# hzxie/RMNet

Measured on AMD Instinct MI355X. Metric: frames/sec at 480p, 1 object, T=5 memory; memory-read HBM GB/s vs peak, higher is better.
Workload: dtype f32 convs; memory read = fp16 operands (K, V, q, P rounded to 11 bits), fp32 accumulate (RMNET_BANK_F16): the frame loop's default for clips with one object -- on one-object 480x854 clips whose masks HAVE a boundary (tests/live_fixture.py) mask IoU vs the CPU path 0.99993-0.99997 and foreground logi

## Files before the change

include/rmnet_hip.h:

```cpp
#ifndef RMNET_HIP_H_
#define RMNET_HIP_H_

#include <stddef.h>
#include <stdint.h>

#ifdef __cplusplus
extern "C" {
#endif

#define RMNET_ABI_VERSION 6

enum {
  RMNET_OK = 0,
  RMNET_E_INVALID_ARG = -1,
  RMNET_E_WORKSPACE = -2,
  RMNET_E_LAUNCH = -3,
  RMNET_E_UNSUPPORTED = -4
};

int rmnet_abi_version(void);
const char *rmnet_error_string(int code);

size_t rmnet_region_map_workspace_bytes(int B, int K, int H, int W);
int rmnet_region_map_f32(const float *mask, int B, int K, int H, int W, float prob_threshold,
// ... 49 lines not shown
                           void *ev_start, void *ev_mid, void *ev_end);
size_t rmnet_bank_read_workspace_bytes(int no, int h, int w);
size_t rmnet_bank_read_workspace_bytes_for(int no, int h, int w, int T);
int rmnet_bank_read_f32(void *bank, int no, int Tcap, int h, int w, int T,
                        const float *q_key, const float *q_val, const int32_t *qry_rects,
                        float *mem_val, void *workspace, size_t workspace_bytes, void *stream,
                        void *ev_start, void *ev_mid, void *ev_end);

int rmnet_rect_mask_f32(const float *x, int n, int C, int T, int h, int w, const int32_t *rects,
                        float *y, void *stream);

int rmnet_channel_affine_f32(const float *x, const float *scale, const float *shift,
                             const float *res, const float *res_scale, const float *res_shift,
                             int relu, long long N, int C, long long HW, float *out, void *stream);

int rmnet_affine_relu_maxpool_f32(const float *x, const float *scale, const float *shift, long long N,
                                  int C, int H, int W, float *out, void *stream);

int rmnet_upsample2x_add_f32(const float *x, const float *skip, long long N, int C, int h, int w,
                             float *out, void *stream);

int rmnet_channel_affine_nhwc_f32(const float *x, const float *scale, const float *shift, const float *res, const float *res_scale,
                                  const float *res_shift, int relu, long long rows, int C, float *out, void *stream);
int rmnet_upsample2x_add_nhwc_f32(const float *x, const float *skip, long long N, int C, int h, int w, float *out, void *stream);
int rmnet_affine_relu_maxpool_nhwc_f32(const float *x, const float *scale, const float *shift, long long N, int C, int H, int W,
                                       float *out, void *stream);

#define RMNET_CONV_RELU_IN 1
#define RMNET_CONV_RELU_OUT 2
int rmnet_conv3x3_split_f32(const float *x, const void *wpack, const float *w_unscale, const float *bias, const float *res, int flags,
                            int N, int H, int W, int Cin, float *out, int32_t *range_word, void *stream);

int rmnet_conv3x3_split_lds_f32(const float *x, const void *wpack, const float *w_unscale, const float *bias, const float *res,
                                int flags, int N, int H, int W, int Cin, float *out, int32_t *range_word, void *stream);

int rmnet_conv3x3_rows_f32(const float *x, const void *wpack, const float *w_unscale, const float *bias, const float *res, int flags,
                           int N, int H, int W, int Cin, float *out, int32_t *range_word, void *stream);

int rmnet_conv_split_f32(const float *x, const void *wpack, const float *w_unscale, const float *shift, const float *res, int flags,
                         int N, int H, int W, int Cin, int Cout, int ksize, int stride, float *out, float *out2, int out_split,
                         int32_t *range_word, void *stream);

#define RMNET_CONV_X_SPLIT 4
#define RMNET_CONV_OUT_SPLIT 8
int rmnet_conv_split_pre_f32(const void *x, const void *wpack, const float *w_unscale, const float *shift, const float *res, int flags,
                             int N, int H, int W, int Cin, int Cout, int ksize, int stride, void *out, float *out2, int out_split,
                             int32_t *range_word, void *stream);
int rmnet_split_act_f32(const float *x, long long M, int C, int relu, void *out, int32_t *range_word, void *stream);

int rmnet_conv_rows_pre_f32(const void *x, const void *wpack, const float *w_unscale, const float *shift, const float *res, int flags,
                            int N, int H, int W, int Cin, int Cout, int ksize, int stride, void *out, float *out2, int out_split,
                            int32_t *range_word, void *stream);

int rmnet_stem_split_f32(const float *frame, const float *mask, const float *other, const void *wpack, const float *w_unscale,
                         const float *shift, int N, int H, int W, float *out, int32_t *range_word, void *stream);

int rmnet_flow_stem_f32(const float *img0, const float *img1, long long batch_stride0, long long batch_stride1, const void *wpack,
                        const float *w_unscale, const float *bias, int N, int H, int W, int Hpad, int Wpad, int lh, int lw, float *out, int32_t *range_word, void *stream);

int rmnet_pred_head_f32(const float *x, const float *w, const float *bias, int n, int Hq, int Wq, int C, float *out, void *stream);

#define RMNET_FLOW_RELU 1
#define RMNET_FLOW_LEAKY 2
#define RMNET_FLOW_TRANSPOSED 4
int rmnet_flow_conv_f32(const float *x, int x_ld, const void *wpack, const float *w_unscale, const float *shift, int flags, int N, int H,
                        int W, int Cin, int Cout, int ksize, int stride, float *out, int out_ld, int coff, int32_t *range_word,
                        void *stream);

size_t rmnet_flow_head_workspace_bytes(int N, int H, int W, int Cin);
int rmnet_flow_head_f32(const float *x, int x_ld, const float *wpack, const float *bias, int N, int H, int W, int Cin, float *out,
                        void *workspace, size_t workspace_bytes, void *stream);

int rmnet_flow_up_f32(const float *flow, const float *w, int N, int h, int w_, float *out, int out_ld, int coff, void *stream);

int rmnet_soft_aggregate_f32(const float *dec, const int32_t *obj_begin, int B, int K, int Hp, int Wp,
                             int pad_l, int pad_t, int H, int W, float *logit, float *prob,
                             void *stream);

int rmnet_flow_affine_f32(const float *flow, const float *m1, const float *m2, int H, int W,
                          float *out, void *stream);
size_t rmnet_flow_affine_workspace_bytes(int H, int W);
int rmnet_flow_affine_f32_host(const float *flow_host, const float *m1_host, const float *m2_host,
                               int H, int W, float *out_host, void *workspace,
                               size_t workspace_bytes, void *stream);

#ifdef __cplusplus
}
#endif
#endif
```

rmnet_amd/_lib.py:

```python

import ctypes
import os

_HERE = os.path.dirname(os.path.abspath(__file__))
LIB_PATH = os.environ.get('RMNET_HIP_LIB') or os.path.join(_HERE, 'librmnet_hip.so')

c_f32p = ctypes.c_void_p
c_i32p = ctypes.c_void_p

SIGNATURES = {
    'rmnet_abi_version': (ctypes.c_int, []),
    'rmnet_error_string': (ctypes.c_char_p, [ctypes.c_int]),
    'rmnet_region_map_workspace_bytes': (ctypes.c_size_t, [ctypes.c_int] * 4),
    'rmnet_region_map_f32': (ctypes.c_int, [
        c_f32p, ctypes.c_int, ctypes.c_int, ctypes.c_int, ctypes.c_int, ctypes.c_float, ctypes.c_int,
        ctypes.c_int, c_f32p, c_i32p, c_i32p, ctypes.c_int, ctypes.c_int, ctypes.c_int, ctypes.c_int,
        ctypes.c_int, ctypes.c_void_p, ctypes.c_size_t, ctypes.c_void_p]),
    'rmnet_region_map_warped_f32': (ctypes.c_int, [
        c_f32p, c_f32p, ctypes.c_int, ctypes.c_int, ctypes.c_int, ctypes.c_int, ctypes.c_float, ctypes.c_int,
        ctypes.c_int, c_f32p, c_i32p, c_i32p, ctypes.c_int, ctypes.c_int, ctypes.c_int, ctypes.c_int,
        ctypes.c_int, c_f32p, ctypes.c_void_p, ctypes.c_size_t, ctypes.c_void_p]),
    'rmnet_boxes_to_cell_rects_i32': (ctypes.c_int, [
        c_i32p, ctypes.c_int, ctypes.c_int, ctypes.c_int, ctypes.c_int, ctypes.c_int, ctypes.c_int,
        ctypes.c_int, c_i32p, ctypes.c_void_p]),
# ... 15 lines not shown
        ctypes.c_void_p, ctypes.c_int, ctypes.c_int, ctypes.c_int, ctypes.c_int, ctypes.c_int, c_f32p,
        c_f32p, c_i32p, ctypes.c_void_p]),
    'rmnet_bank_append_f32_at': (ctypes.c_int, [
        ctypes.c_void_p, ctypes.c_int, ctypes.c_int, ctypes.c_int, ctypes.c_int, ctypes.c_int, c_i32p, c_f32p,
        c_f32p, c_i32p, ctypes.c_void_p]),
    'rmnet_bank_read_f32_at': (ctypes.c_int, [
        ctypes.c_void_p, ctypes.c_int, ctypes.c_int, ctypes.c_int, ctypes.c_int, ctypes.c_int, c_i32p, ctypes.c_int, c_f32p,
        c_f32p, c_i32p, c_f32p, ctypes.c_void_p, ctypes.c_size_t, ctypes.c_void_p, ctypes.c_void_p,
        ctypes.c_void_p, ctypes.c_void_p]),
    'rmnet_bank_read_workspace_bytes': (ctypes.c_size_t, [ctypes.c_int] * 3),
    'rmnet_bank_read_workspace_bytes_for': (ctypes.c_size_t, [ctypes.c_int] * 4),
    'rmnet_bank_read_f32': (ctypes.c_int, [
        ctypes.c_void_p, ctypes.c_int, ctypes.c_int, ctypes.c_int, ctypes.c_int, ctypes.c_int, c_f32p,
        c_f32p, c_i32p, c_f32p, ctypes.c_void_p, ctypes.c_size_t, ctypes.c_void_p, ctypes.c_void_p,
        ctypes.c_void_p, ctypes.c_void_p]),
    'rmnet_rect_mask_f32': (ctypes.c_int, [
        c_f32p, ctypes.c_int, ctypes.c_int, ctypes.c_int, ctypes.c_int, ctypes.c_int, c_i32p, c_f32p,
        ctypes.c_void_p]),
    'rmnet_channel_affine_f32': (ctypes.c_int, [
        c_f32p, c_f32p, c_f32p, c_f32p, c_f32p, c_f32p, ctypes.c_int, ctypes.c_longlong, ctypes.c_int,
        ctypes.c_longlong, c_f32p, ctypes.c_void_p]),
    'rmnet_upsample2x_add_f32': (ctypes.c_int, [
        c_f32p, c_f32p, ctypes.c_longlong, ctypes.c_int, ctypes.c_int, ctypes.c_int, c_f32p, ctypes.c_void_p]),
    'rmnet_soft_aggregate_f32': (ctypes.c_int, [
        c_f32p, c_i32p, ctypes.c_int, ctypes.c_int, ctypes.c_int, ctypes.c_int, ctypes.c_int, ctypes.c_int,
        ctypes.c_int, ctypes.c_int, c_f32p, c_f32p, ctypes.c_void_p]),
    'rmnet_affine_relu_maxpool_f32': (ctypes.c_int, [
        c_f32p, c_f32p, c_f32p, ctypes.c_longlong, ctypes.c_int, ctypes.c_int, ctypes.c_int, c_f32p,
        ctypes.c_void_p]),
    'rmnet_channel_affine_nhwc_f32': (ctypes.c_int, [
        c_f32p, c_f32p, c_f32p, c_f32p, c_f32p, c_f32p, ctypes.c_int, ctypes.c_longlong, ctypes.c_int, c_f32p, ctypes.c_void_p]),
    'rmnet_upsample2x_add_nhwc_f32': (ctypes.c_int, [
        c_f32p, c_f32p, ctypes.c_longlong, ctypes.c_int, ctypes.c_int, ctypes.c_int, c_f32p, ctypes.c_void_p]),
    'rmnet_affine_relu_maxpool_nhwc_f32': (ctypes.c_int, [
        c_f32p, c_f32p, c_f32p, ctypes.c_longlong, ctypes.c_int, ctypes.c_int, ctypes.c_int, c_f32p, ctypes.c_void_p]),
    'rmnet_conv3x3_split_f32': (ctypes.c_int, [
        c_f32p, ctypes.c_void_p, c_f32p, c_f32p, c_f32p, ctypes.c_int, ctypes.c_int, ctypes.c_int, ctypes.c_int, ctypes.c_int,
        c_f32p, c_i32p, ctypes.c_void_p]),
    'rmnet_conv3x3_split_lds_f32': (ctypes.c_int, [
        c_f32p, ctypes.c_void_p, c_f32p, c_f32p, c_f32p, ctypes.c_int, ctypes.c_int, ctypes.c_int, ctypes.c_int, ctypes.c_int,
        c_f32p, c_i32p, ctypes.c_void_p]),
    'rmnet_conv3x3_rows_f32': (ctypes.c_int, [
        c_f32p, ctypes.c_void_p, c_f32p, c_f32p, c_f32p, ctypes.c_int, ctypes.c_int, ctypes.c_int, ctypes.c_int, ctypes.c_int,
        c_f32p, c_i32p, ctypes.c_void_p]),
    'rmnet_conv_split_f32': (ctypes.c_int, [
        c_f32p, ctypes.c_void_p, c_f32p, c_f32p, c_f32p, ctypes.c_int, ctypes.c_int, ctypes.c_int, ctypes.c_int, ctypes.c_int,
        ctypes.c_int, ctypes.c_int, ctypes.c_int, c_f32p, c_f32p, ctypes.c_int, c_i32p, ctypes.c_void_p]),
    'rmnet_conv_split_pre_f32': (ctypes.c_int, [
        ctypes.c_void_p, ctypes.c_void_p, c_f32p, c_f32p, c_f32p, ctypes.c_int, ctypes.c_int, ctypes.c_int, ctypes.c_int, ctypes.c_int,
        ctypes.c_int, ctypes.c_int, ctypes.c_int, ctypes.c_void_p, c_f32p, ctypes.c_int, c_i32p, ctypes.c_void_p]),
    'rmnet_conv_rows_pre_f32': (ctypes.c_int, [
        ctypes.c_void_p, ctypes.c_void_p, c_f32p, c_f32p, c_f32p, ctypes.c_int, ctypes.c_int, ctypes.c_int, ctypes.c_int, ctypes.c_int,
        ctypes.c_int, ctypes.c_int, ctypes.c_int, ctypes.c_void_p, c_f32p, ctypes.c_int, c_i32p, ctypes.c_void_p]),
    'rmnet_split_act_f32': (ctypes.c_int, [
        c_f32p, ctypes.c_longlong, ctypes.c_int, ctypes.c_int, ctypes.c_void_p, c_i32p, ctypes.c_void_p]),
    'rmnet_stem_split_f32': (ctypes.c_int, [
        c_f32p, c_f32p, c_f32p, ctypes.c_void_p, c_f32p, c_f32p, ctypes.c_int, ctypes.c_int, ctypes.c_int, c_f32p, c_i32p,
        ctypes.c_void_p]),
    'rmnet_flow_stem_f32': (ctypes.c_int, [
        c_f32p, c_f32p, ctypes.c_longlong, ctypes.c_longlong, ctypes.c_void_p, c_f32p, c_f32p, ctypes.c_int, ctypes.c_int, ctypes.c_int,
        ctypes.c_int, ctypes.c_int, ctypes.c_int, ctypes.c_int, c_f32p, c_i32p, ctypes.c_void_p]),
    'rmnet_pred_head_f32': (ctypes.c_int, [
        c_f32p, c_f32p, c_f32p, ctypes.c_int, ctypes.c_int, ctypes.c_int, ctypes.c_int, c_f32p, ctypes.c_void_p]),
    'rmnet_flow_conv_f32': (ctypes.c_int, [
        c_f32p, ctypes.c_int, ctypes.c_void_p, c_f32p, c_f32p, ctypes.c_int, ctypes.c_int, ctypes.c_int, ctypes.c_int, ctypes.c_int,
        ctypes.c_int, ctypes.c_int, ctypes.c_int, c_f32p, ctypes.c_int, ctypes.c_int, c_i32p, ctypes.c_void_p]),
    'rmnet_flow_head_workspace_bytes': (ctypes.c_size_t, [ctypes.c_int] * 4),
    'rmnet_flow_head_f32': (ctypes.c_int, [
        c_f32p, ctypes.c_int, c_f32p, c_f32p, ctypes.c_int, ctypes.c_int, ctypes.c_int, ctypes.c_int, c_f32p, ctypes.c_void_p,
        ctypes.c_size_t, ctypes.c_void_p]),
    'rmnet_flow_up_f32': (ctypes.c_int, [
        c_f32p, c_f32p, ctypes.c_int, ctypes.c_int, ctypes.c_int, c_f32p, ctypes.c_int, ctypes.c_int, ctypes.c_void_p]),
    'rmnet_flow_affine_f32': (ctypes.c_int, [
        c_f32p, c_f32p, c_f32p, ctypes.c_int, ctypes.c_int, c_f32p, ctypes.c_void_p]),
    'rmnet_flow_affine_workspace_bytes': (ctypes.c_size_t, [ctypes.c_int, ctypes.c_int]),
    'rmnet_flow_affine_f32_host': (ctypes.c_int, [
        ctypes.c_void_p, ctypes.c_void_p, ctypes.c_void_p, ctypes.c_int, ctypes.c_int,
        ctypes.c_void_p, ctypes.c_void_p, ctypes.c_size_t, ctypes.c_void_p]),
}

ABI_VERSION = 6
_lib = None


class RMNetHipError(RuntimeError):
    pass


def load():
    global _lib
    if _lib is not None:
        return _lib
    if not os.path.exists(LIB_PATH):
        raise RMNetHipError(
            'librmnet_hip.so is missing (%s). The HIP kernels are the only implementation of this '
            'path; build them with `python -m rmnet_amd.build`.' % LIB_PATH)
    lib = ctypes.CDLL(LIB_PATH)
    for name, (res, args) in SIGNATURES.items():
        fn = getattr(lib, name)
        fn.restype = res
        fn.argtypes = args
    if lib.rmnet_abi_version() != ABI_VERSION:
        raise RMNetHipError('librmnet_hip.so ABI %d != expected %d' % (lib.rmnet_abi_version(), ABI_VERSION))
    _lib = lib
    return lib

# ... 6 lines not shown
```

rmnet_amd/build.py:

```python

import os
import shutil
import subprocess

HERE = os.path.dirname(os.path.abspath(__file__))
CSRC = os.path.join(HERE, 'csrc')
SOURCES = ['capi.hip', 'region_map.hip', 'flow_affine.hip', 'memory_read.hip', 'bank.hip', 'epilogue.hip', 'conv3x3.hip', 'conv3x3_rows.hip', 'conv_split.hip',
           'conv_rows.hip', 'stem.hip', 'pred_head.hip', 'flow_conv.hip', 'flow_head.hip', 'flow_stem.hip']
LIB = os.path.join(HERE, 'librmnet_hip.so')
ARCH = 'gfx950'


def hipcc_path():
    for cand in (shutil.which('hipcc'), '/opt/rocm/bin/hipcc'):
        if cand and os.path.exists(cand):
            return cand
    raise RuntimeError('hipcc not found: librmnet_hip.so cannot be built')


def dependencies():
    headers = sorted(f for f in os.listdir(CSRC) if f.endswith('.h'))
    return [os.path.join(CSRC, f) for f in SOURCES + headers] + [os.path.join(os.path.dirname(HERE), 'include', 'rmnet_hip.h')]


def needs_build():
    if not os.path.exists(LIB):
        return True
    t = os.path.getmtime(LIB)
    return any(os.path.getmtime(d) > t for d in dependencies())


def build_library(force=False, verbose=False):
    if not force and not needs_build():
        return LIB
    cmd = [hipcc_path(), '--offload-arch=' + ARCH, '-O3', '-std=c++17', '-shared', '-fPIC',
           '-o', LIB] + [os.path.join(CSRC, s) for s in SOURCES]
    if verbose:
        print(' '.join(cmd))
    subprocess.check_call(cmd, cwd=CSRC)
    return LIB


if __name__ == '__main__':
    print(build_library(force=True, verbose=True))
```

rmnet_amd/csrc/conv_rows_core.h:

```cpp
#pragma once

#include <mutex>

#include "common.h"

namespace rmnet {
namespace {

typedef _Float16 half8 __attribute__((ext_vector_type(8)));
typedef _Float16 half4 __attribute__((ext_vector_type(4)));
typedef float f32x4 __attribute__((ext_vector_type(4)));
typedef unsigned int u32x4 __attribute__((ext_vector_type(4)));

constexpr int kKT = 32;
constexpr int kThreads = 512;
constexpr float kActScale = 64.0f;
constexpr float kActUnscale = 1.0f / 64.0f;
constexpr float kF16Max = 65504.0f;
constexpr int kZeroRows = 4;
constexpr int kAhead = 1;

constexpr int rows_image_bytes(int C, int MT) { return (MT + 2 + kZeroRows) * C * 4; }

__device__ inline int swzr(int row, int chunk) { return row * kKT + ((chunk ^ ((row >> 1) & 2)) << 3); }

__device__ inline void split4(const f32x4 v, half4& hi, half4& lo, int& bad, int count = 1) {
#pragma unroll
  for (int e = 0; e < 4; ++e) {
    const float y = v[e] * kActScale;
    bad += !(fabsf(y) <= kF16Max) ? count : 0;
    const float c = fminf(fmaxf(y, -kF16Max), kF16Max);
    const _Float16 h = (_Float16)c;
    hi[e] = h;
    lo[e] = (_Float16)(c - (float)h);
  }
}

inline bool overlap(const void* p, long long pn, const void* q, long long qn) {
  const char* a = reinterpret_cast<const char*>(p);
  const char* b = reinterpret_cast<const char*>(q);
  return a < b + qn && b < a + pn;
}

extern __shared__ __attribute__((aligned(16))) _Float16 rows_lds[];

template <int C, int MT>
struct RowsCore {
  static constexpr int kCB = C / kKT;
  static constexpr int kStaged = MT + 2;
  static constexpr int kPlaneHalves = (kStaged + kZeroRows) * kKT;
  static constexpr int kBlockHalves = 2 * kPlaneHalves;
  static constexpr int kWPlane = C * kKT;
  static_assert(C % kKT == 0 && kCB % 2 == 0 && MT % 128 == 0 && (MT / 128) * kCB == 8, "8 waves of 128 pixels x 32 channels");
  static_assert(kStaged % 4 == 2, "the zero row of a masked lane: (kStaged + (row + 2) % 4) % 4 == row % 4");
  static_assert(kCB * kBlockHalves * 2 == rows_image_bytes(C, MT), "the image");

  int fr, fc, pix;
  unsigned inside[3];
  half8 wa[4], wb[4];
  const half8* wsrc;
  const half8* wlast;
  unsigned wl;
  f32x4 acc[8][2], accx[8][2];

  __device__ __forceinline__ void begin(int tid, int wcol, int pix_, int m1, const half8* wp, int M, int H, int W) {
    fr = tid & 15, fc = (tid & 63) >> 4, pix = pix_;
    if (tid < 16 * 2 * kCB) *reinterpret_cast<half8*>(rows_lds + (tid >> 4) * kPlaneHalves + kStaged * kKT + 8 * (tid & 15)) = half8{0, 0, 0, 0, 0, 0, 0, 0};
    const int HW = H * W;
    inside[0] = inside[1] = inside[2] = 0u;
#pragma unroll
    for (int i = 0; i < 8; ++i) {
      const int m = m1 + 16 * i + fr;
      const bool pin = m < M;
      const int r = (pin ? m : 0) % HW;
      const int ph = r / W, pw = r % W;
      unsigned bits = 0;
#pragma unroll
      for (int t = 0; t < 9; ++t) {
        const int h = ph + t / 3 - 1, w = pw + t % 3 - 1;
        bits |= (pin && h >= 0 && h < H && w >= 0 && w < W ? 1u : 0u) << t;
      }
      inside[i / 3] |= bits << (9 * (i % 3));
    }
    wsrc = wp;
    wlast = wp + (9 * kCB - 1) * (2 * kWPlane / 8);
    wl = (wcol * 32 + fr) * 4 + fc;
#pragma unroll
    for (int i = 0; i < 8; ++i)
#pragma unroll
      for (int j = 0; j < 2; ++j) acc[i][j] = accx[i][j] = f32x4{0.f, 0.f, 0.f, 0.f};
    load_w(wa);
  }

  __device__ __forceinline__ void load_w(half8 (&w)[4]) {
// ... 5 lines not shown
  }

  __device__ __forceinline__ void run_tap(int tap) {
    const int dx1 = tap % 3;
    unsigned ao[8];
#pragma unroll
    for (int i = 0; i < 8; ++i) {
      const bool in = (inside[i / 3] >> (9 * (i % 3) + tap)) & 1;
      const int row = pix + 16 * i + fr + dx1;
      const unsigned real = (unsigned)swzr(row, fc);
      ao[i] = in ? real : (unsigned)((kStaged + ((row + 2) & 3)) * kKT) + (real & (kKT - 1));
    }
    half8 bh[kAhead + 1], bl[kAhead + 1];
    auto frag = [&](int n) __attribute__((always_inline)) {
      const _Float16* p = rows_lds + ao[n & 7] + (n >> 3) * kBlockHalves;
      bh[n % (kAhead + 1)] = *reinterpret_cast<const half8*>(p);
      bl[n % (kAhead + 1)] = *reinterpret_cast<const half8*>(p + kPlaneHalves);
    };
    auto mma = [&](int cb, const half8(&w)[4]) __attribute__((always_inline)) {
#pragma unroll
      for (int i = 0; i < 8; ++i) {
        if (8 * cb + i + kAhead < 8 * kCB) frag(8 * cb + i + kAhead);
        const half8 h = bh[(8 * cb + i) % (kAhead + 1)], l = bl[(8 * cb + i) % (kAhead + 1)];
#pragma unroll
        for (int j = 0; j < 2; ++j) acc[i][j] = __builtin_amdgcn_mfma_f32_16x16x32_f16(w[2 * j], h, acc[i][j], 0, 0, 0);
#pragma unroll
        for (int j = 0; j < 2; ++j) accx[i][j] = __builtin_amdgcn_mfma_f32_16x16x32_f16(w[2 * j], l, accx[i][j], 0, 0, 0);
#pragma unroll
        for (int j = 0; j < 2; ++j) accx[i][j] = __builtin_amdgcn_mfma_f32_16x16x32_f16(w[2 * j + 1], h, accx[i][j], 0, 0, 0);
      }
    };
    auto step = [&](int cb, const half8(&wc)[4], half8(&wn)[4]) __attribute__((always_inline)) {
      __builtin_amdgcn_sched_barrier(0);
      load_w(wn);
      __builtin_amdgcn_sched_barrier(0);
      mma(cb, wc);
#pragma unroll
      for (int i = 0; i < 8; ++i) {
        __builtin_amdgcn_sched_group_barrier(0x100, 2, 0);
        __builtin_amdgcn_sched_group_barrier(0x008, 6, 0);
      }
    };
#pragma unroll
    for (int n = 0; n < kAhead; ++n) frag(n);
#pragma unroll
    for (int cb = 0; cb < kCB; cb += 2) {
      step(cb, wa, wb);
      step(cb + 1, wb, wa);
    }
    __builtin_amdgcn_sched_barrier(0);
  }

  __device__ __forceinline__ void unscale_shift(const float* unscale, const float* shift, int wcol) {
#pragma unroll
    for (int j = 0; j < 2; ++j) {
      const int co = wcol * 32 + j * 16 + 4 * fc;
      const f32x4 us = *reinterpret_cast<const f32x4*>(unscale + co) * kActUnscale;
      const f32x4 b = shift ? *reinterpret_cast<const f32x4*>(shift + co) : f32x4{0.f, 0.f, 0.f, 0.f};
#pragma unroll
      for (int i = 0; i < 8; ++i) acc[i][j] = (acc[i][j] + accx[i][j]) * us + b;
    }
#pragma unroll
    for (int j = 0; j < 2; ++j)
#pragma unroll
      for (int i = 0; i < 8; ++i) asm volatile("" : "+v"(acc[i][j]));
  }
};

template <auto Kernel, int kBytes>
int rows_prepare(hipStream_t st) {
  static std::mutex mu;
  static bool done[64] = {};
  int dev = 0;
  if (hipGetDevice(&dev) != hipSuccess || dev < 0 || dev >= 64) return RMNET_E_LAUNCH;
  std::lock_guard<std::mutex> lock(mu);
  if (done[dev]) return RMNET_OK;
  hipStreamCaptureStatus cs = hipStreamCaptureStatusNone;
  if (hipStreamIsCapturing(st, &cs) != hipSuccess) return RMNET_E_LAUNCH;
  if (cs != hipStreamCaptureStatusNone) return RMNET_E_UNSUPPORTED;
  if (hipFuncSetAttribute(reinterpret_cast<const void*>(Kernel), hipFuncAttributeMaxDynamicSharedMemorySize, kBytes) != hipSuccess)
    return RMNET_E_LAUNCH;
  done[dev] = true;
  return RMNET_OK;
}

}
}
```

rmnet_amd/networks.py:

```python

import torch
import torch.nn.functional as F
from torch import nn


class _Bottleneck(nn.Module):

    def __init__(self, c_in, width, stride, project):
        super().__init__()
        c_out = width * 4
        self.conv1 = nn.Conv2d(c_in, width, 1, bias=False)
        self.bn1 = nn.BatchNorm2d(width)
        self.conv2 = nn.Conv2d(width, width, 3, stride=stride, padding=1, bias=False)
        self.bn2 = nn.BatchNorm2d(width)
        self.conv3 = nn.Conv2d(width, c_out, 1, bias=False)
        self.bn3 = nn.BatchNorm2d(c_out)
        self.relu = nn.ReLU(inplace=True)
        self.downsample = None
        if project:
            self.downsample = nn.Sequential(nn.Conv2d(c_in, c_out, 1, stride=stride, bias=False),
                                            nn.BatchNorm2d(c_out))

    def forward(self, x):
        if getattr(self, '_fused', False) and not self.training and x.is_cuda:
            return self._forward_fused(x)
        skip = x if self.downsample is None else self.downsample(x)
        y = self.relu(self.bn1(self.conv1(x)))
        y = self.relu(self.bn2(self.conv2(y)))
        y = self.bn3(self.conv3(y))
        return self.relu(y + skip)

    def _forward_fused(self, x):
        from . import ops
        if _split_path_ok(self, x, self.conv1, ('full', 'split', 'trunk')):
            x = x.contiguous(memory_format=torch.channels_last)
            rw = ops.conv_range_word(x.device)
            pre = conv_presplit()
            t = ops.conv_split(x, self._wp1, self._wu1, self._b1, ksize=1, relu_out=True, range_word=rw, out_presplit=pre)
            t = ops.conv_split(t, self._wp2, self._wu2, self._b2, ksize=3, stride=self.conv2.stride[0], relu_out=True, range_word=rw,
                               out_presplit=pre and self.conv3.in_channels >= PRESPLIT_MIN_CIN_1X1)
            if self.downsample is None:
                return ops.conv_split(t, self._wp3, self._wu3, self._b3, res=x, ksize=1, relu_out=True, range_word=rw)
            d = ops.conv_split(x, self._wpd, self._wud, self._bd, ksize=1, stride=self.downsample[0].stride[0], range_word=rw)
            return ops.conv_split(t, self._wp3, self._wu3, self._b3, res=d, ksize=1, relu_out=True, out=d, range_word=rw)
        t = self.conv1(x)
        ops.channel_affine(t, self._s1, self._b1, relu=True, out=t)
        t = self.conv2(t)
        ops.channel_affine(t, self._s2, self._b2, relu=True, out=t)
        t = self.conv3(t)
        if self.downsample is None:
            return ops.channel_affine(t, self._s3, self._b3, res=x, relu=True, out=t)
        d = self.downsample[0](x)
        return ops.channel_affine(t, self._s3, self._b3, res=d, res_scale=self._sd, res_shift=self._bd,
                                  relu=True, out=t)


def _stage(c_in, width, n_blocks, stride):
    blocks = [_Bottleneck(c_in, width, stride, project=True)]
    blocks += [_Bottleneck(width * 4, width, 1, project=False) for _ in range(n_blocks - 1)]
    return nn.Sequential(*blocks)


class ResNet50Trunk(nn.Module):

    def __init__(self):
        super().__init__()
        self.conv1 = nn.Conv2d(3, 64, 7, stride=2, padding=3, bias=False)
        self.bn1 = nn.BatchNorm2d(64)
        self.relu = nn.ReLU(inplace=True)
        self.maxpool = nn.MaxPool2d(3, stride=2, padding=1)
        self.layer1 = _stage(64, 64, 3, 1)
        self.layer2 = _stage(256, 128, 4, 2)
        self.layer3 = _stage(512, 256, 6, 2)


def resnet50(pretrained=False):
    return ResNet50Trunk()


class ResBlock(nn.Module):

    def __init__(self, indim, outdim=None, stride=1):
        super().__init__()
        outdim = indim if outdim is None else outdim
        self.downsample = None
        if not (indim == outdim and stride == 1):
            self.downsample = nn.Conv2d(indim, outdim, 3, padding=1, stride=stride)
        self.conv1 = nn.Conv2d(indim, outdim, 3, padding=1, stride=stride)
        self.conv2 = nn.Conv2d(outdim, outdim, 3, padding=1)

    def forward(self, x):
        if getattr(self, '_fused', False) and not self.training and x.is_cuda:
            return self._forward_fused(x)
        r = self.conv2(F.relu(self.conv1(F.relu(x))))
        return (x if self.downsample is None else self.downsample(x)) + r

    def _forward_fused(self, x):
        from . import ops
        c1, c2 = self.conv1, self.conv2
        if self.downsample is None and _split_conv_ok(self, x, c1) and _split_conv_ok(self, x, c2):
            x = x.contiguous(memory_format=torch.channels_last)
            rw = ops.conv_range_word(x.device)
            t = ops.conv3x3_split(x, self._wp1, self._wu1, c1.bias, relu_in=True, relu_out=True, range_word=rw)
            return ops.conv3x3_split(t, self._wp2, self._wu2, c2.bias, res=x, range_word=rw)
        t = F.conv2d(F.relu(x), c1.weight, None, c1.stride, c1.padding)
        ops.channel_affine(t, None, c1.bias, relu=True, out=t)
        r = F.conv2d(t, c2.weight, None, c2.stride, c2.padding)
        if self.downsample is None:
            return ops.channel_affine(r, None, c2.bias, res=x, out=r)
        ds = self.downsample
        d = F.conv2d(x, ds.weight, None, ds.stride, ds.padding)
        return ops.channel_affine(r, None, c2.bias, res=d, res_shift=ds.bias, out=r)

# ... 389 lines not shown
```

rmnet_amd/ops.py:

```python

import ctypes
import os

import numpy as np
import torch

from . import _lib


MR_FORCE_GENERIC = 1
MR_EXACT_FP32 = 2
BANK_MAX_SLOTS = 2048


def _check(t, name, dtype=torch.float32):
    if not isinstance(t, torch.Tensor):
        raise RuntimeError('%s must be a torch.Tensor' % name)
    if not t.is_cuda:
        raise RuntimeError('%s must be a CUDA tensor' % name)
    if not t.is_contiguous():
        raise RuntimeError('%s must be contiguous' % name)
    if t.dtype != dtype:
        raise RuntimeError('%s must be %s, got %s' % (name, dtype, t.dtype))

# ... 638 lines not shown
    if wpack.numel() != ksize * ksize * cin * cout * 2:
        raise RuntimeError('wpack has %d elements, a %dx%d Cin = %d Cout = %d pack has %d'
                           % (wpack.numel(), ksize, ksize, cin, cout, ksize * ksize * cin * cout * 2))
    pad = ksize // 2
    shape = (N, cout, (H + 2 * pad - ksize) // stride + 1, (W + 2 * pad - ksize) // stride + 1)
    if shift is not None:
        _check(shift, 'shift')
        if shift.numel() != cout:
            raise RuntimeError('shift must have Cout = %d elements' % cout)
    if res is not None:
        _check_act(res, 'res')
        if tuple(res.shape) != shape or not res.is_contiguous(memory_format=torch.channels_last):
            raise RuntimeError('res must be a channels-last %s tensor' % (shape,))
    out2 = None
    if out_presplit:
        if split is not None or out is not None:
            raise RuntimeError('conv_split: out_presplit returns one new split activation, without split / out')
        out = torch.empty((N, shape[2], shape[3], cout // 32, 2, 32), dtype=torch.float16, device=x.device)
    elif split is not None:
        if res is not None or out is not None or not 0 < split < cout or split % 4:
            raise RuntimeError('conv_split: split must be a multiple of 4 in (0, %d), without res / out' % cout)
        out = torch.empty((N, split) + shape[2:], dtype=torch.float32, device=x.device, memory_format=torch.channels_last)
        out2 = torch.empty((N, cout - split) + shape[2:], dtype=torch.float32, device=x.device, memory_format=torch.channels_last)
    elif out is None:
        out = torch.empty(shape, dtype=torch.float32, device=x.device, memory_format=torch.channels_last)
    else:
        _check_act(out, 'out')
        if tuple(out.shape) != shape or not out.is_contiguous(memory_format=torch.channels_last):
            raise RuntimeError('out must be a channels-last %s tensor' % (shape,))
    if range_word is not None:
        _check(range_word, 'range_word', torch.int32)
    for t in (wpack, w_unscale, shift, res, out, range_word):
        if t is not None and t.device != x.device:
            raise RuntimeError('conv_split: every tensor must be on %s' % x.device)
    flags = (CONV_RELU_IN if relu_in else 0) | (CONV_RELU_OUT if relu_out else 0)
    rows = trunk_rows_enabled() and x_split and ksize == 3 and stride == 1 and cin == cout and cin in TRUNK_ROWS_CLASSES \
        and res is None and split is None
    lib = _lib.load()
    with torch.cuda.device(x.device):
        if x_split or out_presplit:
            flags |= (CONV_X_SPLIT if x_split else 0) | (CONV_OUT_SPLIT if out_presplit else 0)
            what = TRUNK_ROWS_ENTRY if rows else 'rmnet_conv_split_pre_f32'
            rc = getattr(lib, what)(_ptr(x), _ptr(wpack), _ptr(w_unscale), _ptr(shift), _ptr(res), flags, N, H, W, cin,
                                    cout, ksize, stride, _ptr(out), _ptr(out2), split or 0, _ptr(range_word),
                                    _stream(x.device))
        else:
            what = 'rmnet_conv_split_f32'
            rc = lib.rmnet_conv_split_f32(_ptr(x), _ptr(wpack), _ptr(w_unscale), _ptr(shift), _ptr(res), flags, N, H, W, cin, cout,
                                          ksize, stride, _ptr(out), _ptr(out2), split or 0, _ptr(range_word), _stream(x.device))
    _lib.check(rc, what)
    return out if out2 is None else (out, out2)


FLOW_RELU, FLOW_LEAKY, FLOW_TRANSPOSED = 1, 2, 4
_FLOW_ACT = {None: 0, False: 0, 'none': 0, True: FLOW_RELU, 'relu': FLOW_RELU, 'leaky': FLOW_LEAKY}


def flow_conv_phase_weights(weight):
    w = weight.permute(1, 0, 2, 3)
    phases = []
    for a in (0, 1):
        for b in (0, 1):
            ky = torch.tensor([3 - a, 1 - a], device=w.device)
            kx = torch.tensor([3 - b, 1 - b], device=w.device)
            phases.append(w.index_select(2, ky).index_select(3, kx))
    return torch.stack(phases, 0)


@torch.no_grad()
def flow_conv_pack(weight, transposed=False):
    if weight.dim() != 4 or weight.shape[2] != weight.shape[3] or weight.shape[2] not in ((4,) if transposed else (3, 5)):
        raise RuntimeError('flow_conv_pack needs a [Cout, Cin, k, k] weight with k in (3, 5), or transposed a [Cin, Cout, 4, 4] one, '
                           'got %s' % (tuple(weight.shape),))
    if weight.dtype != torch.float32:
        raise RuntimeError('flow_conv_pack needs fp32 weights, got %s' % weight.dtype)
    w = weight.detach().double()
    w = flow_conv_phase_weights(w) if transposed else w.unsqueeze(0)
    P, cout, cin, kh, kw = w.shape
    if cout % 64:
        raise RuntimeError('flow_conv_pack needs Cout % 64 == 0, got ' + str(cout))
    cp = (cin + 31) // 32 * 32
    amax = w.abs().amax(dim=(0, 2, 3, 4))
    _, ex = torch.frexp(amax)
    e = torch.where(amax > 0, 15 - ex, torch.zeros_like(ex))
    ws = torch.ldexp(w, e.view(1, -1, 1, 1, 1).to(w.dtype))
    hi = ws.half()
    lo = (ws - hi.double()).half()
    pad = lambda p: torch.nn.functional.pad(p, (0, 0, 0, 0, 0, cp - cin))
    planes = torch.stack([pad(p).reshape(P, cout, cp // 32, 32, kh * kw).permute(0, 4, 2, 1, 3) for p in (hi, lo)], dim=3)
    unscale = torch.ldexp(torch.ones_like(amax), (-e).to(amax.dtype)).float()
    return planes.contiguous().view(-1).view(torch.int16), unscale.contiguous()


def flow_conv_out_hw(H, W, ksize, stride, transposed):
    if transposed:
        return 2 * H, 2 * W
    pad = ksize // 2
    return (H + 2 * pad - ksize) // stride + 1, (W + 2 * pad - ksize) // stride + 1


def flow_conv(x, wpack, w_unscale, shift=None, *, ksize=3, stride=1, transposed=False, act=None, cin=None, out=None, out_coff=0,
              range_word=None):
    _check_act(x, 'x')
    if x.dim() != 4 or not x.is_contiguous(memory_format=torch.channels_last):
        raise RuntimeError('x must be a channels-last [N, C, H, W] tensor')
    if transposed:
# ... 343 lines not shown
```

Before: 655.7.

## Fuse each bottleneck's conv3 with the next block's conv1 in a seam kernel

Adds a HIP kernel that computes one block's 1x1 expand conv3 with residual and ReLU, writes y, and keeps the result as fp16 hi/lo halves in LDS. It then immediately runs the next block's 1x1 reduce conv1 over those halves, emitting the presplit t1. This removes a kernel launch and the round trip of re-reading the wide 4C activation for the next conv1 in each ResNet stage. The stage forward is restructured to chain blocks through this seam for widths 128 and 256. The cost is large LDS use per block, which may lower occupancy, plus serialized GEMMs inside one kernel.

Measured after the change: 661.8, median of 6. About the same (+0.9%).

```diff
diff --git a/include/rmnet_hip.h b/include/rmnet_hip.h
--- a/include/rmnet_hip.h
+++ b/include/rmnet_hip.h
@@ -125,6 +125,10 @@
                             int N, int H, int W, int Cin, int Cout, int ksize, int stride, void *out, float *out2, int out_split,
                             int32_t *range_word, void *stream);
 
+int rmnet_conv_seam_f32(const void *t2, const void *wpack3, const float *w_unscale3, const float *shift3, const float *skip,
+                        const void *wpack1, const float *w_unscale1, const float *shift1, long long M, int C, float *y, void *t1,
+                        int32_t *range_word, void *stream);
+
 int rmnet_stem_split_f32(const float *frame, const float *mask, const float *other, const void *wpack, const float *w_unscale,
                          const float *shift, int N, int H, int W, float *out, int32_t *range_word, void *stream);
 
diff --git a/rmnet_amd/_lib.py b/rmnet_amd/_lib.py
--- a/rmnet_amd/_lib.py
+++ b/rmnet_amd/_lib.py
@@ -91,6 +91,9 @@
     'rmnet_conv_rows_pre_f32': (ctypes.c_int, [
         ctypes.c_void_p, ctypes.c_void_p, c_f32p, c_f32p, c_f32p, ctypes.c_int, ctypes.c_int, ctypes.c_int, ctypes.c_int, ctypes.c_int,
         ctypes.c_int, ctypes.c_int, ctypes.c_int, ctypes.c_void_p, c_f32p, ctypes.c_int, c_i32p, ctypes.c_void_p]),
+    'rmnet_conv_seam_f32': (ctypes.c_int, [
+        ctypes.c_void_p, ctypes.c_void_p, c_f32p, c_f32p, c_f32p, ctypes.c_void_p, c_f32p, c_f32p, ctypes.c_longlong, ctypes.c_int,
+        c_f32p, ctypes.c_void_p, c_i32p, ctypes.c_void_p]),
     'rmnet_split_act_f32': (ctypes.c_int, [
         c_f32p, ctypes.c_longlong, ctypes.c_int, ctypes.c_int, ctypes.c_void_p, c_i32p, ctypes.c_void_p]),
     'rmnet_stem_split_f32': (ctypes.c_int, [
diff --git a/rmnet_amd/build.py b/rmnet_amd/build.py
--- a/rmnet_amd/build.py
+++ b/rmnet_amd/build.py
@@ -6,7 +6,7 @@
 HERE = os.path.dirname(os.path.abspath(__file__))
 CSRC = os.path.join(HERE, 'csrc')
 SOURCES = ['capi.hip', 'region_map.hip', 'flow_affine.hip', 'memory_read.hip', 'bank.hip', 'epilogue.hip', 'conv3x3.hip', 'conv3x3_rows.hip', 'conv_split.hip',
-           'conv_rows.hip', 'stem.hip', 'pred_head.hip', 'flow_conv.hip', 'flow_head.hip', 'flow_stem.hip']
+           'conv_rows.hip', 'conv_seam.hip', 'stem.hip', 'pred_head.hip', 'flow_conv.hip', 'flow_head.hip', 'flow_stem.hip']
 LIB = os.path.join(HERE, 'librmnet_hip.so')
 ARCH = 'gfx950'
 
diff --git a/rmnet_amd/csrc/conv_rows_core.h b/rmnet_amd/csrc/conv_rows_core.h
--- a/rmnet_amd/csrc/conv_rows_core.h
+++ b/rmnet_amd/csrc/conv_rows_core.h
@@ -40,6 +40,23 @@
   const char* a = reinterpret_cast<const char*>(p);
   const char* b = reinterpret_cast<const char*>(q);
   return a < b + qn && b < a + pn;
+}
+
+template <int TI, int TJ>
+__device__ __forceinline__ void unscale_shift_tiles(f32x4 (&acc)[TI][TJ], const f32x4 (&accx)[TI][TJ], const float* unscale, const float* shift,
+                                                    int co0) {
+#pragma unroll
+  for (int j = 0; j < TJ; ++j) {
+    const int co = co0 + j * 16;
+    const f32x4 us = *reinterpret_cast<const f32x4*>(unscale + co) * kActUnscale;
+    const f32x4 b = shift ? *reinterpret_cast<const f32x4*>(shift + co) : f32x4{0.f, 0.f, 0.f, 0.f};
+#pragma unroll
+    for (int i = 0; i < TI; ++i) acc[i][j] = (acc[i][j] + accx[i][j]) * us + b;
+  }
+#pragma unroll
+  for (int j = 0; j < TJ; ++j)
+#pragma unroll
+    for (int i = 0; i < TI; ++i) asm volatile("" : "+v"(acc[i][j]));
 }
 
 extern __shared__ __attribute__((aligned(16))) _Float16 rows_lds[];
@@ -151,18 +168,7 @@
   }
 
   __device__ __forceinline__ void unscale_shift(const float* unscale, const float* shift, int wcol) {
-#pragma unroll
-    for (int j = 0; j < 2; ++j) {
-      const int co = wcol * 32 + j * 16 + 4 * fc;
-      const f32x4 us = *reinterpret_cast<const f32x4*>(unscale + co) * kActUnscale;
-      const f32x4 b = shift ? *reinterpret_cast<const f32x4*>(shift + co) : f32x4{0.f, 0.f, 0.f, 0.f};
-#pragma unroll
-      for (int i = 0; i < 8; ++i) acc[i][j] = (acc[i][j] + accx[i][j]) * us + b;
-    }
-#pragma unroll
-    for (int j = 0; j < 2; ++j)
-#pragma unroll
-      for (int i = 0; i < 8; ++i) asm volatile("" : "+v"(acc[i][j]));
+    unscale_shift_tiles<8, 2>(acc, accx, unscale, shift, wcol * 32 + 4 * fc);
   }
 };
 
diff --git a/rmnet_amd/csrc/conv_seam.hip b/rmnet_amd/csrc/conv_seam.hip
--- /dev/null
+++ b/rmnet_amd/csrc/conv_seam.hip
@@ -0,0 +1,254 @@
+#include "conv_rows_core.h"
+
+namespace rmnet {
+namespace {
+
+constexpr int kSeamMT = 64;
+constexpr int kSeamChunk = 256;
+
+template <int C>
+struct Seam {
+  static constexpr int kCB = C / kKT;
+  static constexpr int kChunks = 4 * C / kSeamChunk;
+  static constexpr int kSB = kSeamChunk / kKT;
+  static constexpr int kPlane = kSeamMT * kKT;
+  static constexpr int kBlock = 2 * kPlane;
+  static constexpr int kT2Halves = kCB * kBlock;
+  static constexpr int kBytes = (kCB + kSB) * kBlock * 2;
+  static constexpr int kWC = C >= 128 ? 8 : 4;
+  static constexpr int kWP = 8 / kWC;
+  static constexpr int kTI = 4 / kWP;
+  static constexpr int kTJ = C / (16 * kWC);
+  static_assert(kCB % 2 == 0 && kSB % 2 == 0, "the two weight sets change roles in pairs of steps");
+  static_assert(kWP * kTI * 16 == kSeamMT && kWC * kTJ * 16 == C, "GEMM2's waves cover 64 pixels x C channels");
+  static_assert(kBytes == kSeamMT * C * 4 + 65536 && kBytes <= kLdsBytesPerCU, "LDS budget");
+};
+
+struct SeamArgs {
+  const _Float16* t2;
+  const half8* wp3;
+  const float* unscale3;
+  const float* shift3;
+  const float* skip;
+  const half8* wp1;
+  const float* unscale1;
+  const float* shift1;
+  float* y;
+  _Float16* t1;
+  int* range;
+  int M;
+};
+
+template <int TI, int TJ, int kPlane>
+__device__ __forceinline__ void seam_mma(const _Float16* img, const half8 (&w)[4], f32x4 (&acc)[TI][TJ], f32x4 (&accx)[TI][TJ]) {
+#pragma unroll
+  for (int i = 0; i < TI; ++i) {
+    const half8 h = *reinterpret_cast<const half8*>(img + i * 16 * kKT);
+    const half8 l = *reinterpret_cast<const half8*>(img + kPlane + i * 16 * kKT);
+#pragma unroll
+    for (int j = 0; j < TJ; ++j) acc[i][j] = __builtin_amdgcn_mfma_f32_16x16x32_f16(w[2 * j], h, acc[i][j], 0, 0, 0);
+#pragma unroll
+    for (int j = 0; j < TJ; ++j) accx[i][j] = __builtin_amdgcn_mfma_f32_16x16x32_f16(w[2 * j], l, accx[i][j], 0, 0, 0);
+#pragma unroll
+    for (int j = 0; j < TJ; ++j) accx[i][j] = __builtin_amdgcn_mfma_f32_16x16x32_f16(w[2 * j + 1], h, accx[i][j], 0, 0, 0);
+  }
+  __builtin_amdgcn_sched_group_barrier(0x100, TI > 1 ? 4 : 2, 0);
+#pragma unroll
+  for (int i = 0; i < TI; ++i) {
+    __builtin_amdgcn_sched_group_barrier(0x008, 3 * TJ, 0);
+    if (i + 2 < TI) __builtin_amdgcn_sched_group_barrier(0x100, 2, 0);
+  }
+}
+
+__device__ __forceinline__ unsigned opaque(unsigned v) {
+  asm volatile("" : "+v"(v));
+  return v;
+}
+
+template <int C>
+__global__ __launch_bounds__(kThreads) void conv_seam(SeamArgs a) {
+  using S = Seam<C>;
+  constexpr int CB = S::kCB, kPlane = S::kPlane, kBlock = S::kBlock, TI = S::kTI, TJ = S::kTJ;
+  constexpr int C4 = 4 * C;
+  _Float16* const t2i = rows_lds;
+  _Float16* const yi = rows_lds + S::kT2Halves;
+  const int tid = threadIdx.x, wave = tid >> 6, fr = tid & 15, fc = (tid & 63) >> 4;
+  const int m0 = blockIdx.x * kSeamMT;
+
+  {
+    constexpr int kPassRows = 2 * (kThreads / 16) / CB;
+    static_assert(kPassRows % 8 == 0 && kPassRows * CB == kSeamMT, "a pass keeps the swizzle bit; CB passes stage 64 rows");
+    const int sch = tid & 3, spl = (tid >> 3) & 1, sblk = (tid >> 4) % CB;
+    const int srow = 2 * ((tid >> 4) / CB) + ((tid >> 2) & 1);
+    const unsigned scol = sblk * (2 * kKT) + spl * kKT + 8 * sch;
+    _Float16* const sdst = t2i + sblk * kBlock + spl * kPlane + swzr(srow, sch);
+    u32x4 v[CB];
+#pragma unroll
+    for (int k = 0; k < CB; ++k) {
+      const int q = min(m0 + srow + kPassRows * k, a.M - 1);
+      v[k] = *reinterpret_cast<const u32x4*>(a.t2 + ((unsigned)q * (unsigned)(2 * C) + scol));
+    }
+#pragma unroll
+    for (int k = 0; k < CB; ++k) *reinterpret_cast<u32x4*>(sdst + kPassRows * k * kKT) = v[k];
+  }
+
+  const int wc2 = wave % S::kWC, wp2 = wave / S::kWC;
+  const int co2 = wc2 * 16 * TJ, px2 = wp2 * 16 * TI;
+  const int fo = swzr(fr, fc);
+  int foy = S::kT2Halves + px2 * kKT + fo;
+  asm volatile("" : "+v"(foy));
+  const unsigned wl3 = (32 * wave + fr) * 4 + fc, wl1 = (co2 + fr) * 4 + fc;
+  half8 wa[4], wb[4];
+  auto load3 = [&](half8 (&w)[4], int k, int cb) __attribute__((always_inline)) {
+#pragma unroll
+    for (int j = 0; j < 2; ++j)
+#pragma unroll
+      for (int p = 0; p < 2; ++p) w[2 * j + p] = (a.wp3 + (k * (kSeamChunk * 4) + cb * (C4 * 8) + p * (C4 * 4)))[wl3 + (unsigned)(j * 64)];
+  };
+  auto load1 = [&](half8 (&w)[4], int s) __attribute__((always_inline)) {
+#pragma unroll
+    for (int j = 0; j < TJ; ++j)
+#pragma unroll
+      for (int p = 0; p < 2; ++p) w[2 * j + p] = (a.wp1 + (s * (C * 8) + p * (C * 4)))[wl1 + (unsigned)(j * 64)];
+  };
+  unsigned ro[4];
+#pragma unroll
+  for (int i = 0; i < 4; ++i) ro[i] = (unsigned)(min(i * 16 + fr, a.M - 1 - m0) * C4 + wave * 32 + 4 * fc);
+
+  f32x4 acc[4][2], accx[4][2];
+  f32x4 acc2[TI][TJ], accx2[TI][TJ];
+#pragma unroll
+  for (int i = 0; i < TI; ++i)
+#pragma unroll
+    for (int j = 0; j < TJ; ++j) acc2[i][j] = accx2[i][j] = f32x4{0.f, 0.f, 0.f, 0.f};
+  int bad = 0;
+  load3(wa, 0, 0);
+  __syncthreads();
+
+#pragma unroll 1
+  for (int k = 0; k < S::kChunks; ++k) {
+    f32x4 r[4][2];
+    const float* const skp = a.skip + ((size_t)m0 * C4 + k * kSeamChunk);
+    float* const yp = a.y + ((size_t)m0 * C4 + k * kSeamChunk);
+#pragma unroll
+    for (int i = 0; i < 4; ++i)
+#pragma unroll
+      for (int j = 0; j < 2; ++j) r[i][j] = *reinterpret_cast<const f32x4*>(skp + (opaque(ro[i]) + (unsigned)(j * 16)));
+#pragma unroll
+    for (int i = 0; i < 4; ++i)
+#pragma unroll
+      for (int j = 0; j < 2; ++j) acc[i][j] = accx[i][j] = f32x4{0.f, 0.f, 0.f, 0.f};
+
+#pragma unroll
+    for (int cb = 0; cb < CB; cb += 2) {
+      __builtin_amdgcn_sched_barrier(0);
+      load3(wb, k, cb + 1);
+      __builtin_amdgcn_sched_barrier(0);
+      seam_mma<4, 2, kPlane>(t2i + cb * kBlock + fo, wa, acc, accx);
+      __builtin_amdgcn_sched_barrier(0);
+      if (cb + 2 < CB) load3(wa, k, cb + 2); else load1(wa, k * S::kSB);
+      __builtin_amdgcn_sched_barrier(0);
+      seam_mma<4, 2, kPlane>(t2i + (cb + 1) * kBlock + fo, wb, acc, accx);
+    }
+    __builtin_amdgcn_sched_barrier(0);
+
+    unscale_shift_tiles<4, 2>(acc, accx, a.unscale3, a.shift3, k * kSeamChunk + wave * 32 + 4 * fc);
+    __syncthreads();
+#pragma unroll
+    for (int j = 0; j < 2; ++j) {
+#pragma unroll
+      for (int i = 0; i < 4; ++i) {
+        const int m = m0 + i * 16 + fr;
+        f32x4 v = acc[i][j];
+        v += r[i][j];
+#pragma unroll
+        for (int e = 0; e < 4; ++e) v[e] = v[e] < 0.0f ? 0.0f : v[e];
+        if (m < a.M) *reinterpret_cast<f32x4*>(yp + (opaque(ro[i]) + (unsigned)(j * 16))) = v;
+        half4 hi, lo;
+        split4(v, hi, lo, bad, m < a.M ? 1 : 0);
+        _Float16* o = yi + wave * kBlock + swzr(i * 16 + fr, 2 * j + (fc >> 1)) + 4 * (fc & 1);
+        *reinterpret_cast<half4*>(o) = hi;
+        *reinterpret_cast<half4*>(o + kPlane) = lo;
+      }
+    }
+    __syncthreads();
+
+    const int kn = k + 1 < S::kChunks ? k + 1 : k;
+#pragma unroll
+    for (int s = 0; s < S::kSB; s += 2) {
+      __builtin_amdgcn_sched_barrier(0);
+      load1(wb, k * S::kSB + s + 1);
+      __builtin_amdgcn_sched_barrier(0);
+      seam_mma<TI, TJ, kPlane>(rows_lds + s * kBlock + foy, wa, acc2, accx2);
+      __builtin_amdgcn_sched_barrier(0);
+      if (s + 2 < S::kSB) load1(wa, k * S::kSB + s + 2); else load3(wa, kn, 0);
+      __builtin_amdgcn_sched_barrier(0);
+      seam_mma<TI, TJ, kPlane>(rows_lds + (s + 1) * kBlock + foy, wb, acc2, accx2);
+    }
+    __builtin_amdgcn_sched_barrier(0);
+  }
+
+  unscale_shift_tiles<TI, TJ>(acc2, accx2, a.unscale1, a.shift1, co2 + 4 * fc);
+#pragma unroll
+  for (int j = 0; j < TJ; ++j) {
+    const int co = co2 + j * 16 + 4 * fc;
+#pragma unroll
+    for (int i = 0; i < TI; ++i) {
+      const int m = m0 + px2 + i * 16 + fr;
+      if (m >= a.M) continue;
+      f32x4 v = acc2[i][j];
+#pragma unroll
+      for (int e = 0; e < 4; ++e) v[e] = v[e] < 0.0f ? 0.0f : v[e];
+      half4 hi, lo;
+      split4(v, hi, lo, bad);
+      _Float16* o = a.t1 + (size_t)m * (2 * C) + (co >> 5) * (2 * kKT) + (co & 31);
+      *reinterpret_cast<half4*>(o) = hi;
+      *reinterpret_cast<half4*>(o + kKT) = lo;
+    }
+  }
+  if (a.range && bad) atomicAdd(a.range, bad);
+}
+
+template <int C>
+int seam_launch(const SeamArgs& a, hipStream_t st) {
+  const int rc = rows_prepare<conv_seam<C>, Seam<C>::kBytes>(st);
+  if (rc != RMNET_OK) return rc;
+  hipLaunchKernelGGL((conv_seam<C>), dim3((unsigned)((a.M + kSeamMT - 1) / kSeamMT)), dim3(kThreads), Seam<C>::kBytes, st, a);
+  return check_launch();
+}
+
+}
+}
+
+extern "C" int rmnet_conv_seam_f32(const void* t2, const void* wpack3, const float* w_unscale3, const float* shift3, const float* skip,
+                                   const void* wpack1, const float* w_unscale1, const float* shift1, long long M, int C, float* y, void* t1,
+                                   int32_t* range_word, void* stream) {
+  using namespace rmnet;
+  if (!t2 || !wpack3 || !w_unscale3 || !skip || !wpack1 || !w_unscale1 || !y || !t1 || M <= 0) return RMNET_E_INVALID_ARG;
+  if ((reinterpret_cast<uintptr_t>(t2) | reinterpret_cast<uintptr_t>(wpack3) | reinterpret_cast<uintptr_t>(w_unscale3) |
+       reinterpret_cast<uintptr_t>(shift3) | reinterpret_cast<uintptr_t>(skip) | reinterpret_cast<uintptr_t>(wpack1) |
+       reinterpret_cast<uintptr_t>(w_unscale1) | reinterpret_cast<uintptr_t>(shift1) | reinterpret_cast<uintptr_t>(y) |
+       reinterpret_cast<uintptr_t>(t1)) & 15)
+    return RMNET_E_INVALID_ARG;
+  if (reinterpret_cast<uintptr_t>(range_word) & 3) return RMNET_E_INVALID_ARG;
+  if (C != 64 && C != 128 && C != 256) return RMNET_E_UNSUPPORTED;
+  if (M >= (1LL << 31) / (4 * C)) return RMNET_E_UNSUPPORTED;
+  const long long nb = M * C * 4, wb = 2LL * C * 4 * C * 2;
+  const struct { const void* p; long long n; } in[] = {{t2, nb}, {wpack3, wb}, {w_unscale3, 16LL * C}, {shift3, shift3 ? 16LL * C : 0},
+                                                        {wpack1, wb}, {w_unscale1, 4LL * C}, {shift1, shift1 ? 4LL * C : 0},
+                                                        {range_word, range_word ? 4 : 0}};
+  for (const auto& t : in) {
+    if (!t.n) continue;
+    if (overlap(y, 4 * nb, t.p, t.n) || overlap(t1, nb, t.p, t.n)) return RMNET_E_INVALID_ARG;
+  }
+  if (y != skip && overlap(y, 4 * nb, skip, 4 * nb)) return RMNET_E_INVALID_ARG;
+  if (overlap(t1, nb, skip, 4 * nb) || overlap(t1, nb, y, 4 * nb)) return RMNET_E_INVALID_ARG;
+  SeamArgs a;
+  a.t2 = reinterpret_cast<const _Float16*>(t2); a.wp3 = reinterpret_cast<const half8*>(wpack3); a.unscale3 = w_unscale3; a.shift3 = shift3;
+  a.skip = skip; a.wp1 = reinterpret_cast<const half8*>(wpack1); a.unscale1 = w_unscale1; a.shift1 = shift1; a.y = y;
+  a.t1 = reinterpret_cast<_Float16*>(t1); a.range = range_word; a.M = (int)M;
+  hipStream_t st = (hipStream_t)stream;
+  if (C == 256) return seam_launch<256>(a, st);
+  if (C == 128) return seam_launch<128>(a, st);
+  return seam_launch<64>(a, st);
+}
diff --git a/rmnet_amd/networks.py b/rmnet_amd/networks.py
--- a/rmnet_amd/networks.py
+++ b/rmnet_amd/networks.py
@@ -36,13 +36,9 @@
             x = x.contiguous(memory_format=torch.channels_last)
             rw = ops.conv_range_word(x.device)
             pre = conv_presplit()
-            t = ops.conv_split(x, self._wp1, self._wu1, self._b1, ksize=1, relu_out=True, range_word=rw, out_presplit=pre)
-            t = ops.conv_split(t, self._wp2, self._wu2, self._b2, ksize=3, stride=self.conv2.stride[0], relu_out=True, range_word=rw,
-                               out_presplit=pre and self.conv3.in_channels >= PRESPLIT_MIN_CIN_1X1)
-            if self.downsample is None:
-                return ops.conv_split(t, self._wp3, self._wu3, self._b3, res=x, ksize=1, relu_out=True, range_word=rw)
-            d = ops.conv_split(x, self._wpd, self._wud, self._bd, ksize=1, stride=self.downsample[0].stride[0], range_word=rw)
-            return ops.conv_split(t, self._wp3, self._wu3, self._b3, res=d, ksize=1, relu_out=True, out=d, range_word=rw)
+            t = self._split_head(x, rw, pre)
+            t, skip, out = self._split_body(x, t, rw, pre and self.conv3.in_channels >= PRESPLIT_MIN_CIN_1X1)
+            return self._split_tail(t, skip, out, rw)
         t = self.conv1(x)
         ops.channel_affine(t, self._s1, self._b1, relu=True, out=t)
         t = self.conv2(t)
@@ -54,11 +50,67 @@
         return ops.channel_affine(t, self._s3, self._b3, res=d, res_scale=self._sd, res_shift=self._bd,
                                   relu=True, out=t)
 
+    def _split_head(self, x, rw, pre):
+        from . import ops
+        return ops.conv_split(x, self._wp1, self._wu1, self._b1, ksize=1, relu_out=True, range_word=rw, out_presplit=pre)
+
+    def _split_body(self, x, t, rw, t2_split):
+        from . import ops
+        t = ops.conv_split(t, self._wp2, self._wu2, self._b2, ksize=3, stride=self.conv2.stride[0], relu_out=True, range_word=rw,
+                           out_presplit=t2_split)
+        if self.downsample is None:
+            return t, x, None
+        d = ops.conv_split(x, self._wpd, self._wud, self._bd, ksize=1, stride=self.downsample[0].stride[0], range_word=rw)
+        return t, d, d
+
+    def _split_tail(self, t, skip, out, rw):
+        from . import ops
+        return ops.conv_split(t, self._wp3, self._wu3, self._b3, res=skip, ksize=1, relu_out=True, out=out, range_word=rw)
+
+
+class _Stage(nn.Sequential):
+
+    def _seam_ok(self, x):
+        from . import ops
+        blocks = list(self)
+        if len(blocks) < 2 or not all(isinstance(b, _Bottleneck) for b in blocks):
+            return False
+        b0 = blocks[0]
+        if not _split_path_ok(b0, x, b0.conv1, ('full', 'split', 'trunk')):
+            return False
+        width = b0.conv3.in_channels
+        s = b0.conv2.stride[0]
+        if ((x.shape[2] - 1) // s + 1) * ((x.shape[3] - 1) // s + 1) == 1:
+            return False
+        for b in blocks[1:]:
+            if not (getattr(b, '_fused', False) and getattr(b, '_conv_split', False)) or b.training or b.downsample is not None:
+                return False
+            if b.conv1.in_channels != 4 * width or b.conv3.in_channels != width or b.conv2.stride != (1, 1):
+                return False
+        return conv_presplit() and ops.trunk_seam_enabled() and width in ops.TRUNK_SEAM_CLASSES
+
+    def forward(self, x):
+        if not self._seam_ok(x):
+            for b in self:
+                x = b(x)
+            return x
+        from . import ops
+        blocks = list(self)
+        x = x.contiguous(memory_format=torch.channels_last)
+        rw = ops.conv_range_word(x.device)
+        t = blocks[0]._split_head(x, rw, True)
+        for b, nxt in zip(blocks, blocks[1:] + [None]):
+            if nxt is None:
+                t, skip, out = b._split_body(x, t, rw, b.conv3.in_channels >= PRESPLIT_MIN_CIN_1X1)
+                return b._split_tail(t, skip, out, rw)
+            t, skip, out = b._split_body(x, t, rw, True)
+            x, t = ops.conv_seam(t, b._wp3, b._wu3, b._b3, skip, nxt._wp1, nxt._wu1, nxt._b1, out=out, range_word=rw)
+
 
 def _stage(c_in, width, n_blocks, stride):
     blocks = [_Bottleneck(c_in, width, stride, project=True)]
     blocks += [_Bottleneck(width * 4, width, 1, project=False) for _ in range(n_blocks - 1)]
-    return nn.Sequential(*blocks)
+    return _Stage(*blocks)
 
 
 class ResNet50Trunk(nn.Module):
diff --git a/rmnet_amd/ops.py b/rmnet_amd/ops.py
--- a/rmnet_amd/ops.py
+++ b/rmnet_amd/ops.py
@@ -714,6 +714,60 @@
     return out if out2 is None else (out, out2)
 
 
+TRUNK_SEAM_DEFAULT = True
+TRUNK_SEAM_ENTRY = 'rmnet_conv_seam_f32'
+TRUNK_SEAM_ALL = (64, 128, 256)
+TRUNK_SEAM_CLASSES = (128, 256)
+
+
+def trunk_seam_enabled():
+    v = os.environ.get('RMNET_TRUNK_SEAM')
+    if v is None:
+        return TRUNK_SEAM_DEFAULT
+    if v.strip() not in ('0', '1'):
+        raise RuntimeError("RMNET_TRUNK_SEAM must be '0' or '1', got %r" % v)
+    return v.strip() == '1'
+
+
+def conv_seam(t2, wpack3, w_unscale3, shift3, skip, wpack1, w_unscale1, shift1, out=None, range_word=None):
+    _check_split_act(t2, 't2')
+    N, H, W = t2.shape[:3]
+    C = t2.shape[3] * 32
+    if C not in TRUNK_SEAM_ALL or t2.numel() == 0:
+        raise RuntimeError('conv_seam needs C in %s and a non-empty tensor, got %s' % (TRUNK_SEAM_ALL, tuple(t2.shape)))
+    shape = (N, 4 * C, H, W)
+    for t, n, dt, numel in ((wpack3, 'wpack3', torch.int16, 8 * C * C), (wpack1, 'wpack1', torch.int16, 8 * C * C),
+                            (w_unscale3, 'w_unscale3', torch.float32, 4 * C), (w_unscale1, 'w_unscale1', torch.float32, C),
+                            (shift3, 'shift3', torch.float32, 4 * C), (shift1, 'shift1', torch.float32, C)):
+        if t is None and n.startswith('shift'):
+            continue
+        _check(t, n, dt)
+        if t.numel() != numel:
+            raise RuntimeError('%s has %d elements, a C = %d seam needs %d' % (n, t.numel(), C, numel))
+    _check_act(skip, 'skip')
+    if tuple(skip.shape) != shape or not skip.is_contiguous(memory_format=torch.channels_last):
+        raise RuntimeError('skip must be a channels-last %s tensor' % (shape,))
+    if out is None:
+        out = torch.empty(shape, dtype=torch.float32, device=t2.device, memory_format=torch.channels_last)
+    else:
+        _check_act(out, 'out')
+        if tuple(out.shape) != shape or not out.is_contiguous(memory_format=torch.channels_last):
+            raise RuntimeError('out must be a channels-last %s tensor' % (shape,))
+    if range_word is not None:
+        _check(range_word, 'range_word', torch.int32)
+    for t in (wpack3, w_unscale3, shift3, skip, wpack1, w_unscale1, shift1, out, range_word):
+        if t is not None and t.device != t2.device:
+            raise RuntimeError('conv_seam: every tensor must be on %s' % t2.device)
+    t1 = torch.empty((N, H, W, C // 32, 2, 32), dtype=torch.float16, device=t2.device)
+    lib = _lib.load()
+    with torch.cuda.device(t2.device):
+        rc = getattr(lib, TRUNK_SEAM_ENTRY)(_ptr(t2), _ptr(wpack3), _ptr(w_unscale3), _ptr(shift3), _ptr(skip), _ptr(wpack1),
+                                            _ptr(w_unscale1), _ptr(shift1), N * H * W, C, _ptr(out), _ptr(t1), _ptr(range_word),
+                                            _stream(t2.device))
+    _lib.check(rc, TRUNK_SEAM_ENTRY)
+    return out, t1
+
+
 FLOW_RELU, FLOW_LEAKY, FLOW_TRANSPOSED = 1, 2, 4
 _FLOW_ACT = {None: 0, False: 0, 'none': 0, True: FLOW_RELU, 'relu': FLOW_RELU, 'leaky': FLOW_LEAKY}
 
```
